# WilliamFlinchbaugh/Deep-RL-Battlespace

Measured on AMD Instinct MI355X. Metric: agent-steps/sec, higher is better.
Workload: dtype f64/i16

## Files before the change

### deep-rl-battlespace_amd/build.py

```python
import os
import subprocess
import sys

HERE = os.path.dirname(os.path.abspath(__file__))
CSRC = os.path.join(HERE, "csrc")
INCLUDE = os.path.join(os.path.dirname(HERE), "include")
LIB = os.path.join(CSRC, "libbattlespace_hip.so")
COMMON = ["-O3", "--offload-arch=gfx950", "-fPIC", "-std=c++17", "-Wall", "-Wno-unused-function"]
STEP_FLAGS = ["-ffp-contract=off", "-mllvm", "-disable-machine-licm", "-mllvm", "-amdgpu-mfma-vgpr-form", "-mllvm", "-amdgpu-kernarg-preload-count=15"]
PER_CALL_FLAGS = STEP_FLAGS + ["-mllvm", "-amdgpu-sched-strategy=max-ilp"]
SOURCES = [(os.path.join(CSRC, "bsx_kernels.hip"), STEP_FLAGS),
           (os.path.join(CSRC, "bsx_step_per_call.hip"), PER_CALL_FLAGS),
           (os.path.join(CSRC, "bsx_step_multi_tick.hip"), STEP_FLAGS),
           (os.path.join(CSRC, "bsx_step_two_wave.hip"), PER_CALL_FLAGS),
           (os.path.join(CSRC, "bsx_step_rollout.hip"), STEP_FLAGS),
           (os.path.join(CSRC, "bsx_actor.hip"), ["-ffp-contract=off", "-mllvm", "-amdgpu-mfma-vgpr-form"]),
           (os.path.join(CSRC, "bsx_actor_grad.hip"), ["-ffp-contract=off", "-mllvm", "-amdgpu-mfma-vgpr-form"]),
           (os.path.join(CSRC, "bsx_replay.hip"), []),
           (os.path.join(CSRC, "bsx_advantage.hip"), ["-ffp-contract=off"]),
           (os.path.join(CSRC, "bsx_ppo_head.hip"), []),
           (os.path.join(CSRC, "bsx_adam_step.hip"), [])]


def _stale():
    if not os.path.exists(LIB):
        return True
    t = os.path.getmtime(LIB)
    import glob
    deps = [src for src, _ in SOURCES] + glob.glob(os.path.join(CSRC, "*.h")) + glob.glob(os.path.join(CSRC, "*.inl")) + \
        [os.path.join(INCLUDE, "battlespace_hip.h"), os.path.abspath(__file__)]
    return any(os.path.getmtime(d) > t for d in deps)


def build(force=False, verbose=False):
    if not force and not _stale():
        return LIB
    hipcc = os.environ.get("HIPCC", "/opt/rocm/bin/hipcc")
    from concurrent.futures import ThreadPoolExecutor

    def compile_one(item):
        src, extra = item
        obj = os.path.splitext(src)[0] + ".o"
        cmd = [hipcc, *COMMON, *extra, "-I", INCLUDE, "-c", src, "-o", obj]
        if verbose:
            print(" ".join(cmd), flush=True)
        subprocess.run(cmd, check=True)
        return obj
    with ThreadPoolExecutor(max_workers=len(SOURCES)) as pool:
        objs = list(pool.map(compile_one, SOURCES))
    cmd = [hipcc, "--offload-arch=gfx950", "-shared", "-fPIC", *objs, "-o", LIB]
    if verbose:
        print(" ".join(cmd), flush=True)
    subprocess.run(cmd, check=True)
    return LIB


if __name__ == "__main__":
    print(build(force="--force" in sys.argv, verbose=True))
```

### deep-rl-battlespace_amd/csrc/bsx_kernels.hip

```cpp

#include <array>
#include <mutex>
#include <unordered_map>

#include "bsx_config.h"
#include "bsx_args.h"
#include "bsx_state.h"
#include "bsx_rng.h"
#include "bsx_geometry.h"
#include "bsx_instinct.h"
#include "bsx_step_kernel.h"
#define BSX_INST_PER_CALL
#define BSX_INST_MULTI_TICK
#define BSX_INST_ROLLOUT
#include "bsx_step_split.h"
#define BSX_INST_SPLIT_MANY
#define BSX_INST_SPLIT
#define BSX_INST_SPLIT_CONT
#ifdef BSX_VARIANT
#define BSX_INST_KW
#else
#define BSX_INST_KW extern
#endif
#include "bsx_step_instances.h"
using namespace bsxk;

namespace {

struct ResetArgs {
    StatePtrs st; int64_t E; int n; const uint8_t* mask; const int32_t* spawn; uint64_t seed; uint64_t nonce;
    int64_t env_offset; float* obs; int observe_only;
};

__global__ __launch_bounds__(TPB) void bsx_reset_kernel(const ResetArgs p) {
    const int n = p.n, A = 2 * n, G = group_width(n), EPB = TPB / G;
    const int tid = threadIdx.x, a = tid & (G - 1), gl = tid & ~(G - 1);
    const int64_t e = int64_t(blockIdx.x) * EPB + (tid / G);
    const bool env_ok = e < p.E, valid = env_ok && a < A;
    const size_t g = valid ? size_t(e) * A + a : 0;
    __shared__ volatile int s_x[TPB], s_y[TPB], s_hp[TPB];

    EnvU er = {};
    uint32_t games = 0;
    int x = 0, y = 0, hp = 0;
    double dir = 0.0;
    bool frac = false;
    if (env_ok) {
        const uint2 dw = p.st.envd[e];
        er = unpack_env(p.st.envc[e], dw.x);
        games = dw.y;
    }
    if (valid) {
        const uint2 pw = p.st.plane[g];
        unpack_plane(pw, x, y, hp, dir);
        frac = (pw.y & PLANE_FRAC) != 0u;
        if (frac) dir = p.st.pdirf[g];
    }
    const bool doit = env_ok && !p.observe_only && (!p.mask || p.mask[e]);
    if (p.spawn) {
        if (doit) {
            const int32_t* s = p.spawn + size_t(e) * (4 + 3 * A);
            er.brx = s[0]; er.bry = s[1]; er.bbx = s[2]; er.bby = s[3];
            if (valid) { x = s[4 + 3 * a]; y = s[5 + 3 * a]; dir = double(s[6 + 3 * a]); }
        }
    } else if (!p.observe_only) {
        const int64_t genv = p.env_offset + (env_ok ? e : p.E - 1);
        const int ac = a < A ? a : A - 1;
        const SpawnDraw sd = spawn_from_words(draw4(p.seed, genv, STREAM_RESET, uint32_t(p.nonce), uint32_t(ac)), ac, n);
        const int lane0 = (tid & 63) & ~(G - 1);
        const int rbx = __shfl(sd.bx, lane0), rby = __shfl(sd.by, lane0), bbx = __shfl(sd.bx, lane0 + n), bby = __shfl(sd.by, lane0 + n);
        if (doit) {
            er.brx = rbx; er.bry = rby; er.bbx = bbx; er.bby = bby;
            if (valid) { x = sd.x; y = sd.y; dir = double(sd.dir); }
        }
    }
    if (doit) {
        er.bhp_r = er.bhp_b = 5 * n;
        er.tick = 0; er.done = 0; er.winner = BSX_WINNER_NONE;
        hp = PLANE_HP; frac = false;
        if (valid) p.st.plane[g] = pack_plane(x, y, hp, dir, false);
        if (valid && a == 0) { p.st.envc[e] = pack_envc(er); p.st.envd[e] = make_uint2(pack_envd(er), games); }
    }
    if (!p.observe_only) {
        const int lane = tid & 63;
        const int64_t wb = int64_t(blockIdx.x) * (TPB / 64) + (tid >> 6);
        const unsigned long long resetting = __ballot(doit);
        if (resetting != 0ull && wb < wave_blocks(p.E, n)) {
            uint2* const pool = p.st.bent + size_t(wb) * POOL_CAP;
            const int pc = int(p.st.bcnt[wb]);
            int wpos = 0;
            for (int base = 0; base < pc; base += 64) {
                const int w = base + lane;
                const uint2 en = pool[w < pc ? w : 0];
                const bool stay = w < pc && ((resetting >> (en.x >> ENT_OWNER_SHIFT)) & 1ull) == 0ull;
                const unsigned long long kb = __ballot(stay);
                const int ps = wpos + __popcll(kb & ((1ull << lane) - 1ull));
                if (stay) pool[ps] = en;
                wpos += __popcll(kb);
            }
            if (lane == 0) p.st.bcnt[wb] = uint32_t(wpos);
        }
    }
    s_x[tid] = x; s_y[tid] = y; s_hp[tid] = valid ? hp : 0;
    __syncthreads();
    if (valid && p.obs) {
        const int team = a < n ? 0 : 1;
        write_obs<0>(p.obs + g * size_t(3 * n + 2), n, hp > 0, x, y, dir, a,
                     team == 0 ? er.bbx : er.brx, team == 0 ? er.bby : er.bry, gl, s_x, s_y, s_hp);
    }
}

__global__ void bsx_mark_done_kernel(uint2* envd, int64_t E) {
    const int64_t e = int64_t(blockIdx.x) * blockDim.x + threadIdx.x;
    if (e < E) envd[e] = make_uint2(1u << 27, 0u);
}

struct ExportArgs { StatePtrs st; int64_t E; int n; BsxExport out; int tie_tick; };

__global__ __launch_bounds__(TPB) void bsx_export_kernel(const ExportArgs p) {
    const int A = 2 * p.n;
    const size_t EA = size_t(p.E) * A;
    const size_t g = size_t(blockIdx.x) * TPB + threadIdx.x;
    if (g >= EA) return;
    const int64_t e = int64_t(g / A);
    const int a = int(g % A);
    const uint2 pw = p.st.plane[g];
    int x, y, hp;
    double dir;
    unpack_plane(pw, x, y, hp, dir);
    if (pw.y & PLANE_FRAC) dir = p.st.pdirf[g];
    const BsxExport& o = p.out;
    if (o.px) o.px[g] = x;
    if (o.py) o.py[g] = y;
    if (o.pdir) o.pdir[g] = dir;
    if (o.php) o.php[g] = hp;
    if (o.palive) o.palive[g] = hp > 0;
    const uint2 dw = p.st.envd[e];
    const EnvU ev = unpack_env(p.st.envc[e], dw.x);
    const int ptick = ev.tick - ((ev.done && ev.winner == BSX_WINNER_TIE && ev.tick >= p.tie_tick) ? 1 : 0);
    for (int k = 0; k < K; ++k) {
        const size_t i = g * K + k;
        if (o.bl_live) o.bl_live[i] = 0;
        if (o.bl_x) o.bl_x[i] = 0;
        if (o.bl_y) o.bl_y[i] = 0;
        if (o.bl_dir) o.bl_dir[i] = 0.0;
    }
    const int G = group_width(p.n), EPB = 64 / G;
    const int64_t wb = e / EPB;
    const uint32_t me = uint32_t(int(e % EPB) * G + a);
    const uint2* const pool = p.st.bent + size_t(wb) * POOL_CAP;
    const int cnt = int(p.st.bcnt[wb]);
    for (int j2 = 0; j2 < cnt; ++j2) {
        const uint32_t w = pool[j2].x;
        const int age = bullet_age(w);
        if ((w >> ENT_OWNER_SHIFT) != me || age == int(TOMBSTONE_AGE)) continue;
        int slot = (ptick - age + 1) % K;
        if (slot < 0) slot += K;
        const size_t i = g * K + slot;
        if (o.bl_live) o.bl_live[i] = 1;
        if (o.bl_x) o.bl_x[i] = bullet_x(w);
        if (o.bl_y) o.bl_y[i] = bullet_y(w);
        if (o.bl_dir) o.bl_dir[i] = p.st.bdir[size_t(slot) * EA + g];
    }
    if (a == 0) {
        if (o.base_xy) { o.base_xy[4 * e] = ev.brx; o.base_xy[4 * e + 1] = ev.bry; o.base_xy[4 * e + 2] = ev.bbx; o.base_xy[4 * e + 3] = ev.bby; }
        if (o.bhp) { o.bhp[2 * e] = ev.bhp_r; o.bhp[2 * e + 1] = ev.bhp_b; }
        if (o.tick) o.tick[e] = ev.tick;
        if (o.env_done) o.env_done[e] = ev.done;
        if (o.winner) o.winner[e] = ev.winner;
        if (o.counters) {
            const int* c4 = p.st.cnt + 4 * e;
            o.counters[4 * e] = c4[0]; o.counters[4 * e + 1] = c4[1]; o.counters[4 * e + 2] = c4[2]; o.counters[4 * e + 3] = c4[3];
        }
    }
}

struct InstinctArgs {
    const float* obs; void* actions; const double* rnd; int64_t E; int n; int team; int out_kind; int continuous;
    uint64_t seed; uint64_t seq; const uint64_t* seq_base; int64_t env_offset;
};

__global__ __launch_bounds__(TPB) void bsx_instinct_kernel(const InstinctArgs p) {
    const int A = 2 * p.n, D = 3 * p.n + 2;
    const size_t g = size_t(blockIdx.x) * TPB + threadIdx.x;
    if (g >= size_t(p.E) * A) return;
    const int a = int(g % A);
    const int tm = a < p.n ? 0 : 1;
    if (p.team != 2 && p.team != tm) return;
    const float* o = p.obs + g * D;
    double td, ta;
    const int act = instinct_choose([&](int k) { return o[k]; }, p.n, td, ta);
    if (!p.continuous) {
        if (p.out_kind == BSX_ACT_I32) static_cast<int32_t*>(p.actions)[g] = act;
        else static_cast<float4*>(p.actions)[g] = one_hot_scores(act);
        return;
    }
    double r0, n0, n1, n2;
    if (p.rnd) { r0 = p.rnd[4 * g]; n0 = p.rnd[4 * g + 1]; n1 = p.rnd[4 * g + 2]; n2 = p.rnd[4 * g + 3]; }
    else instinct_continuous_draws(p.seed, p.seq + (p.seq_base ? *p.seq_base : 0ull), uint64_t(p.env_offset) * uint64_t(A) + g, r0, n0, n1, n2);
    double* out = static_cast<double*>(p.actions) + 3 * g;
    instinct_continuous_action(td, ta, r0, n0, n1, n2, out[0], out[1], out[2]);
}

std::mutex g_family_mu;
std::unordered_map<const void*, int> g_family;
inline void family_forget(const void* state) {
    std::lock_guard<std::mutex> lk(g_family_mu);
    g_family.erase(state);
}
inline bool family_claim(const void* state, bool cont) {
    std::lock_guard<std::mutex> lk(g_family_mu);
    int& f = g_family[state];
    if (f == 0) f = cont ? 2 : 1;
    return f == (cont ? 2 : 1);
}
inline int grid_for(int64_t E, int n) {
    const int epb = TPB / group_width(n);
    return int((E + epb - 1) / epb);
}

inline bool narrow_offsets_ok(int64_t E, int n, uint32_t flags) {
    return !(flags & BSX_F_WIDE_OFFSETS) && uint64_t(E) * uint64_t(2 * n) * 200ull <= 0xFFFFFFFFull;
}
constexpr int64_t SPLIT_MAX_GAMES = 114688, SPLIT_MANY_MAX_GAMES = 65536, SPLIT_CONT_MAX_GAMES = 81920;
constexpr int64_t SPLIT_DRAW_MAX_GAMES = 98304;
constexpr int64_t SPLIT_MANY_FORM2_FROM = 32768;
template <bool CONT, bool MULTI>
inline bool split_applies(int n, const StepArgs& a, int64_t bound) {
    if (n != 1 || (a.flags & BSX_F_ONE_WAVE)) return false;
    if (CONT) return !MULTI && bound <= SPLIT_CONT_MAX_GAMES;
    return bound <= (MULTI ? SPLIT_MANY_MAX_GAMES : SPLIT_MAX_GAMES);
}

using StepKernel = void (*)(BSX_STEP_KERNEL_PARAMS);

template <class F>
StepKernel by_team_and_offsets(int n, bool off32, F f) {
    const auto w = [&](auto N) { return off32 ? f(N, std::true_type{}) : f(N, std::false_type{}); };
    switch (n) {
        case 1: return w(std::integral_constant<int, 1>{});
        case 2: return w(std::integral_constant<int, 2>{});
        case 3: return w(std::integral_constant<int, 3>{});
        case 4: return w(std::integral_constant<int, 4>{});
        default: return w(std::integral_constant<int, 0>{});
    }
}

template <bool CONT, bool MULTI, bool ACTOR, bool LG>
int launch_for_n(const StepArgs& a, int64_t bound, void* stream) {
    const int n = a.n;
    const bool two_wave = !ACTOR && split_applies<CONT, MULTI>(n, a, bound);
    const StepKernel k = by_team_and_offsets(n, narrow_offsets_ok(a.E, n, a.flags), [&](auto N_, auto OFF32_) -> StepKernel {
        constexpr int N = decltype(N_)::value;
        constexpr bool OFF32 = decltype(OFF32_)::value;
        if constexpr (ACTOR) {
            if constexpr (N == 0) return nullptr;
            else return bsx_step_kernel<N, CONT, true, true, false, OFF32>;
        } else {
            if constexpr (N == 1 && !(CONT && MULTI)) {
                if (two_wave) {
                    if constexpr (MULTI)
                        return bound > SPLIT_MANY_FORM2_FROM ? bsx_step_split_kernel<LG, OFF32, 2>
                                                             : bsx_step_split_kernel<LG, OFF32, 1>;
                    else if constexpr (CONT)
                        return bsx_step_split_kernel<false, OFF32, 0, true, true>;
                    else
                        return bound <= SPLIT_DRAW_MAX_GAMES ? bsx_step_split_kernel<LG, OFF32, 0, false, true>
                                                             : bsx_step_split_kernel<LG, OFF32, 0>;
                }
            }
            return bsx_step_kernel<N, CONT, MULTI, false, LG, OFF32>;
        }
    });
    const StepGeometry geo = step_geometry(ACTOR ? FORM_ROLLOUT : (two_wave ? FORM_TWO_WAVE : FORM_ONE_WAVE), bound, n);
    const dim3 grid(unsigned(geo.groups));
    const dim3 block(SPB * geo.waves);
    hipLaunchKernelGGL(k, grid, block, 0, static_cast<hipStream_t>(stream),
                       bound, a.st.envc, a.st.envd, a.st.plane, a.actions, a.st.bent, a.st.bcnt, a.action_kind, a);
    return int(hipGetLastError());
}

StepArgs step_args(void* state, int64_t E, int n, int T, float* rew, uint8_t* done, uint8_t* env_done, uint8_t* winner,
                   uint8_t* env_done_t, const BsxRewards* cfg, uint32_t flags, uint64_t seed, int64_t env_offset) {
    StepArgs a{};
    a.st = state_ptrs(state, E, n);
    a.E = E; a.n = n; a.T = T;
    a.rew = rew; a.done = done; a.env_done = env_done; a.winner = winner; a.env_done_t = env_done_t;
    a.cfg = *cfg; a.flags = flags; a.seed = seed; a.env_offset = env_offset; a.tie_tick = tie_tick_const(n);
    a.scripted_team = -1;
    return a;
}

struct StepCall { int64_t first = 0, count = -1; int T = 0; int store_all = 0; uint8_t* env_done_t = nullptr; };

template <bool CONT>
int step(const StepCall& c, void* state, int64_t E, int n, const void* actions, int action_kind, const double* u, float* obs, float* rew,
         uint8_t* done, uint8_t* env_done, uint8_t* winner, const BsxRewards* cfg, uint32_t flags, uint64_t seed, int64_t env_offset,
         void* stream) {
    const int T = c.T;
    const int64_t first = c.first, count = c.count < 0 ? E - first : c.count;
    if (T < 0 || T > BSX_MAX_T || first < 0 || count <= 0 || first > E - count || (first & 255) || ((first || count != E) && T != 0))
        return BSX_E_ARG;
    if (!obs || !rew || !done || !cfg || (!actions && (T || !(flags & BSX_F_EMPTY_CALL)))) return BSX_E_ARG;
    if (const int rc = check_games(state, E, n)) return rc;
    if (!aligned(obs, 4) || !aligned(rew, 4) || (u && !aligned(u, 8))) return BSX_E_ALIGN;
    if (!CONT && action_kind == BSX_ACT_LOGITS_F32 && !aligned(actions, 16)) return BSX_E_ALIGN;
    if (!CONT && action_kind != BSX_ACT_I32 && action_kind != BSX_ACT_LOGITS_F32) return BSX_E_ARG;
    if (CONT && action_kind != BSX_ACT_F32 && action_kind != BSX_ACT_F64 && action_kind != BSX_ACT_F32X4) return BSX_E_ARG;
    if (CONT && action_kind == BSX_ACT_F32X4 && !aligned(actions, 16)) return BSX_E_ALIGN;
    if (!family_claim(state, CONT)) return BSX_E_FAMILY;
    StepArgs a = step_args(state, E, n, T, rew, done, env_done, winner, c.env_done_t, cfg, flags, seed, env_offset);
    a.actions = actions; a.action_kind = action_kind; a.u = u; a.obs = obs;
    if (!actions) { a.actions = state; a.action_kind = -1; }
    const int64_t EA = E * 2 * n;
    a.act_tb = EA * (CONT ? (action_kind == BSX_ACT_F32 ? 12 : (action_kind == BSX_ACT_F64 ? 24 : 16)) : (action_kind == BSX_ACT_I32 ? 4 : 16));
    a.u_ts = EA;
    a.obs_ts = c.store_all ? EA * (3 * n + 2) : 0; a.rew_ts = c.store_all ? EA : 0; a.done_ts = c.store_all ? EA : 0;
    if (first) {
        const int64_t fa = first * 2 * n;
        const int64_t fb = first / (64 / group_width(n));
        a.st.envc += first; a.st.envd += first; a.st.cnt += 4 * first; a.st.plane += fa; a.st.pdirf += fa;
        a.st.bcnt += fb; a.st.bent += fb * POOL_CAP; a.st.bdir += fa; a.st.bd += fa;
        if (actions) a.actions = static_cast<const char*>(actions) + fa * (a.act_tb / EA);
        if (u) a.u += fa;
        a.obs += fa * (3 * n + 2); a.rew += fa; a.done += fa;
        if (env_done) a.env_done += first;
        if (winner) a.winner += first;
        a.env_offset += first;
    }
    const bool lg = !CONT && action_kind == BSX_ACT_LOGITS_F32;
    if (T == 0) return lg ? launch_for_n<CONT, false, false, !CONT>(a, count, stream) : launch_for_n<CONT, false, false, false>(a, count, stream);
    return lg ? launch_for_n<CONT, true, false, !CONT>(a, count, stream) : launch_for_n<CONT, true, false, false>(a, count, stream);
}

template <bool CONT>
int rollout(void* state, int64_t E, int n, int T, const float* weights, int precision, int scripted_team, uint64_t scripted_seed, float* obs,
            float* scores, float* rew, uint8_t* done, uint8_t* env_done, uint8_t* winner, uint8_t* env_done_t, const BsxRewards* cfg,
            uint32_t flags, const BsxActorNoise* noise, uint64_t actor_seed, uint64_t seq, const uint64_t* seq_base, uint64_t seed,
            int64_t env_offset, void* stream, bool gauss = false, const BsxGaussianHead* head = nullptr) {
    if (T < 1 || T > BSX_MAX_T || !weights || !obs || !scores || !rew || !done || !cfg || (flags & BSX_F_EMPTY_CALL) ||
        (precision != BSX_ACTOR_F32 && precision != BSX_ACTOR_BF16X3 && precision != BSX_ACTOR_BF16X6) || scripted_team < -1 || scripted_team > 1)
        return BSX_E_ARG;
    if (gauss && (!head || !head->log_std)) return BSX_E_ARG;
    if (const int rc = check_games(state, E, n, 256, ROLLOUT_MAX_N)) return rc;
    if (!aligned(weights, 16) || !aligned(scores, 16) || !aligned(obs, 4) || !aligned(rew, 4)) return BSX_E_ALIGN;
    BsxActorNoise nz = {};
    if (noise) nz = *noise;
    if (gauss) {
        if (nz.gaussian_std > 0.f || nz.ou_scale > 0.f || nz.sample_mode != 0 || nz.u_inject || nz.logp) return BSX_E_ARG;
        if (!aligned(head->log_std, 4) || (head->logp && !aligned(head->logp, 4))) return BSX_E_ALIGN;
    }
    if (nz.ou_scale > 0.f && (!nz.ou_state || !aligned(nz.ou_state, 16))) return nz.ou_state ? BSX_E_ALIGN : BSX_E_ARG;
    if (nz.z_inject || nz.u_inject) return BSX_E_ARG;
    if (nz.sample_mode != 0 && (nz.sample_mode != 1 || !(nz.temperature > 0.f) || CONT)) return BSX_E_ARG;
    if ((nz.logp && !aligned(nz.logp, 4)) || (nz.value_weights && !aligned(nz.value_weights, 16))) return BSX_E_ALIGN;
    if (nz.value_weights && (n != 1 || !nz.value || !aligned(nz.value, 4))) return BSX_E_ARG;
    if (!family_claim(state, CONT)) return BSX_E_FAMILY;
    const int64_t EA = E * 2 * n, D = 3 * n + 2;
    StepArgs a = step_args(state, E, n, T, rew, done, env_done, winner, env_done_t, cfg, flags, seed, env_offset);
    a.action_kind = CONT ? BSX_ACT_F32X4 : BSX_ACT_LOGITS_F32;
    a.obs = obs + EA * D; a.obs_ts = EA * D; a.rew_ts = EA; a.done_ts = EA;
    a.aw = weights; a.aprec = precision; a.scripted_team = scripted_team; a.obs0 = obs; a.scores = scores; a.scores_ts = EA * 4; a.nz = nz;
    a.aseed = actor_seed; a.aseq = seq; a.aseq_base = seq_base; a.iseed = scripted_seed;
    if (gauss) a.gh = *head;
    return launch_for_n<CONT, true, true, false>(a, E, stream);
}

const std::array<double2, 361>& heading_table() {
    static const std::array<double2, 361> lut = [] {
        std::array<double2, 361> t;
        const double st = 215 * 0.1;
        for (int d = 0; d <= 360; ++d) {
            const double ang = -(double(d) * DEG2RAD);
            t[d].x = st * cos(ang);
            t[d].y = st * sin(ang);
        }
        return t;
    }();
    return lut;
}

}

extern "C" {

int bsx_abi_version(void) { return BSX_ABI_VERSION; }

int bsx_build_flags(void) { return BUILD_FLAGS; }

int bsx_stream_synchronize(void* stream) { return int(hipStreamSynchronize(static_cast<hipStream_t>(stream))); }

int bsx_host_device_pointer(void* host, void** device) {
    if (!host || !device) return BSX_E_ARG;
    return int(hipHostGetDevicePointer(device, host, 0));
}

int bsx_tie_tick(int n) { return tie_tick_const(n); }

int bsx_state_bytes(int64_t E, int n, size_t* bytes) {
    if (const int rc = check_games(bytes, E, n, 1)) return rc;
    *bytes = make_layout(E, n).total;
    return 0;
}

int bsx_state_init(void* state, int64_t E, int n, void* stream) {
    if (const int rc = check_games(state, E, n)) return rc;
    const Layout L = make_layout(E, n);
    family_forget(state);
    hipStream_t s = static_cast<hipStream_t>(stream);
    hipError_t err = hipMemsetAsync(state, 0, L.total, s);
    if (err != hipSuccess) return int(err);
    const std::array<double2, 361>& lut = heading_table();
    err = hipMemcpyAsync(static_cast<char*>(state) + L.lut, lut.data(), sizeof(double2) * lut.size(), hipMemcpyHostToDevice, s);
    if (err != hipSuccess) return int(err);
    hipLaunchKernelGGL(bsx_mark_done_kernel, dim3(unsigned((E + TPB - 1) / TPB)), dim3(TPB), 0, s,
                       reinterpret_cast<uint2*>(static_cast<char*>(state) + L.envd), E);
    return int(hipGetLastError());
}

int bsx_state_release(void* state) {
    if (!state) return BSX_E_ARG;
    family_forget(state);
    return 0;
}

int bsx_reset(void* state, int64_t E, int n, const uint8_t* reset_mask, const int32_t* spawn, uint64_t seed,
              uint64_t nonce, int64_t env_offset, float* obs, void* stream) {
    if (const int rc = check_games(state, E, n)) return rc;
    if ((spawn && !aligned(spawn, 4)) || (obs && !aligned(obs, 4))) return BSX_E_ALIGN;
    if (!reset_mask) family_forget(state);
    ResetArgs a{state_ptrs(state, E, n), E, n, reset_mask, spawn, seed, nonce, env_offset, obs, 0};
    hipLaunchKernelGGL(bsx_reset_kernel, dim3(grid_for(E, n)), dim3(TPB), 0, static_cast<hipStream_t>(stream), a);
    return int(hipGetLastError());
}

int bsx_step_discrete(void* state, int64_t E, int n, const void* actions, int action_kind, const double* u, float* obs,
                      float* rew, uint8_t* done, uint8_t* env_done, uint8_t* winner, const BsxRewards* cfg,
                      uint32_t flags, uint64_t seed, int64_t env_offset, void* stream) {
    return step<false>({}, state, E, n, actions, action_kind, u, obs, rew, done, env_done, winner, cfg, flags, seed, env_offset, stream);
}

int bsx_step_continuous(void* state, int64_t E, int n, const void* actions, int action_kind, const double* u,
                        float* obs, float* rew, uint8_t* done, uint8_t* env_done, uint8_t* winner,
                        const BsxRewards* cfg, uint32_t flags, uint64_t seed, int64_t env_offset, void* stream) {
    return step<true>({}, state, E, n, actions, action_kind, u, obs, rew, done, env_done, winner, cfg, flags, seed, env_offset, stream);
}

int bsx_step_discrete_range(void* state, int64_t E, int n, int64_t first, int64_t count, const void* actions, int action_kind, const double* u,
                            float* obs, float* rew, uint8_t* done, uint8_t* env_done, uint8_t* winner, const BsxRewards* cfg,
                            uint32_t flags, uint64_t seed, int64_t env_offset, void* stream) {
    return step<false>({first, count}, state, E, n, actions, action_kind, u, obs, rew, done, env_done, winner, cfg, flags, seed, env_offset, stream);
}

int bsx_step_continuous_range(void* state, int64_t E, int n, int64_t first, int64_t count, const void* actions, int action_kind, const double* u,
                              float* obs, float* rew, uint8_t* done, uint8_t* env_done, uint8_t* winner, const BsxRewards* cfg,
                              uint32_t flags, uint64_t seed, int64_t env_offset, void* stream) {
    return step<true>({first, count}, state, E, n, actions, action_kind, u, obs, rew, done, env_done, winner, cfg, flags, seed, env_offset, stream);
}

int bsx_step_many_discrete(void* state, int64_t E, int n, int T, const void* actions, int action_kind, const double* u,
                           float* obs, float* rew, uint8_t* done, uint8_t* env_done, uint8_t* winner, uint8_t* env_done_t, const BsxRewards* cfg,
                           uint32_t flags, int store_all, uint64_t seed, int64_t env_offset, void* stream) {
    return T < 1 ? BSX_E_ARG : step<false>({0, -1, T, store_all, env_done_t}, state, E, n, actions, action_kind, u, obs, rew, done, env_done,
                                           winner, cfg, flags, seed, env_offset, stream);
}

int bsx_step_many_continuous(void* state, int64_t E, int n, int T, const void* actions, int action_kind, const double* u,
                             float* obs, float* rew, uint8_t* done, uint8_t* env_done, uint8_t* winner, uint8_t* env_done_t, const BsxRewards* cfg,
                             uint32_t flags, int store_all, uint64_t seed, int64_t env_offset, void* stream) {
    return T < 1 ? BSX_E_ARG : step<true>({0, -1, T, store_all, env_done_t}, state, E, n, actions, action_kind, u, obs, rew, done, env_done,
                                          winner, cfg, flags, seed, env_offset, stream);
}

int bsx_rollout_discrete(void* state, int64_t E, int n, int T, const float* weights, int precision, int scripted_team, float* obs, float* scores, float* rew,
                         uint8_t* done, uint8_t* env_done, uint8_t* winner, uint8_t* env_done_t, const BsxRewards* cfg, uint32_t flags,
                         const BsxActorNoise* noise, uint64_t actor_seed, uint64_t seq, const uint64_t* seq_base, uint64_t seed,
                         int64_t env_offset, void* stream) {
    return rollout<false>(state, E, n, T, weights, precision, scripted_team, 0, obs, scores, rew, done, env_done, winner, env_done_t, cfg, flags,
                          noise, actor_seed, seq, seq_base, seed, env_offset, stream);
}

int bsx_rollout_continuous(void* state, int64_t E, int n, int T, const float* weights, int precision, int scripted_team, uint64_t scripted_seed, float* obs, float* scores, float* rew,
                           uint8_t* done, uint8_t* env_done, uint8_t* winner, uint8_t* env_done_t, const BsxRewards* cfg, uint32_t flags,
                           const BsxActorNoise* noise, uint64_t actor_seed, uint64_t seq, const uint64_t* seq_base, uint64_t seed,
                           int64_t env_offset, void* stream) {
    return rollout<true>(state, E, n, T, weights, precision, scripted_team, scripted_seed, obs, scores, rew, done, env_done, winner, env_done_t, cfg, flags,
                         noise, actor_seed, seq, seq_base, seed, env_offset, stream);
}

int bsx_rollout_continuous_gaussian(void* state, int64_t E, int n, int T, const float* weights, int precision, int scripted_team,
                                    uint64_t scripted_seed, float* obs, float* scores, float* rew,
                                    uint8_t* done, uint8_t* env_done, uint8_t* winner, uint8_t* env_done_t, const BsxRewards* cfg,
                                    uint32_t flags, const BsxActorNoise* noise, const BsxGaussianHead* head, uint64_t actor_seed,
                                    uint64_t seq, const uint64_t* seq_base, uint64_t seed, int64_t env_offset, void* stream) {
    return rollout<true>(state, E, n, T, weights, precision, scripted_team, scripted_seed, obs, scores, rew, done, env_done, winner, env_done_t, cfg, flags,
                         noise, actor_seed, seq, seq_base, seed, env_offset, stream, true, head);
}

__global__ void bsx_selftest_atan2_kernel(int R, unsigned long long* out) {
    const int W = 2 * R + 1;
    const long long total = (long long)W * W;
    unsigned long long bad = 0, seen = 0;
    for (long long i = (long long)blockIdx.x * blockDim.x + threadIdx.x; i < total; i += (long long)gridDim.x * blockDim.x) {
        const int iy = int(i / W) - R, ix = int(i % W) - R;
        const double lib = atan2(double(iy), double(ix));
        const double one = atan2_pixels(iy, ix);
        const int ys[3] = {iy, ix, -iy}, xs[3] = {ix, iy, ix};
        double three[3];
        atan2_pixels_n<3>(ys, xs, three);
        const bool ok = __double_as_longlong(one) == __double_as_longlong(lib) && __double_as_longlong(three[0]) == __double_as_longlong(lib) &&
                        __double_as_longlong(three[1]) == __double_as_longlong(atan2(double(ix), double(iy))) &&
                        __double_as_longlong(three[2]) == __double_as_longlong(atan2(double(-iy), double(ix)));
        bad += ok ? 0ull : 1ull;
        seen += 1ull;
    }
    atomicAdd(&out[0], bad); atomicAdd(&out[1], seen);
}
int bsx_selftest_atan2(int R, uint64_t* out, void* stream) {
    if (!out || R < 0 || R > 4096) return BSX_E_ARG;
    hipStream_t st = static_cast<hipStream_t>(stream);
    hipError_t err = hipMemsetAsync(out, 0, 2 * sizeof(uint64_t), st);
    if (err != hipSuccess) return int(err);
    bsx_selftest_atan2_kernel<<<1024, 256, 0, st>>>(R, reinterpret_cast<unsigned long long*>(out));
    return int(hipGetLastError());
}

int bsx_observe(void* state, int64_t E, int n, float* obs, void* stream) {
    if (!obs) return BSX_E_ARG;
    if (const int rc = check_games(state, E, n)) return rc;
    if (!aligned(obs, 4)) return BSX_E_ALIGN;
    ResetArgs a{state_ptrs(state, E, n), E, n, nullptr, nullptr, 0, 0, 0, obs, 1};
    hipLaunchKernelGGL(bsx_reset_kernel, dim3(grid_for(E, n)), dim3(TPB), 0, static_cast<hipStream_t>(stream), a);
    return int(hipGetLastError());
}

int bsx_export_state(const void* state, int64_t E, int n, const BsxExport* out, void* stream) {
    if (!out) return BSX_E_ARG;
    if (const int rc = check_games(state, E, n)) return rc;
    ExportArgs a{state_ptrs(const_cast<void*>(state), E, n), E, n, *out, bsx_tie_tick(n)};
    const size_t EA = size_t(E) * 2 * n;
    hipLaunchKernelGGL(bsx_export_kernel, dim3(unsigned((EA + TPB - 1) / TPB)), dim3(TPB), 0,
                       static_cast<hipStream_t>(stream), a);
    return int(hipGetLastError());
}

int bsx_instinct_discrete(const float* obs, void* actions, int out_kind, int64_t E, int n, int team, void* stream) {
    if (!actions || team < 0 || team > 2 || (out_kind != BSX_ACT_I32 && out_kind != BSX_ACT_LOGITS_F32)) return BSX_E_ARG;
    if (const int rc = check_games(obs, E, n, 4)) return rc;
    if (!aligned(actions, out_kind == BSX_ACT_I32 ? 4 : 16)) return BSX_E_ALIGN;
    InstinctArgs a{obs, actions, nullptr, E, n, team, out_kind, 0, 0, 0, nullptr, 0};
    const size_t EA = size_t(E) * 2 * n;
    hipLaunchKernelGGL(bsx_instinct_kernel, dim3(unsigned((EA + TPB - 1) / TPB)), dim3(TPB), 0, static_cast<hipStream_t>(stream), a);
    return int(hipGetLastError());
}

int bsx_instinct_continuous_shard(const float* obs, double* actions, const double* rnd, int64_t E, int n, int team,
                                  uint64_t seed, uint64_t seq, const uint64_t* seq_base, int64_t env_offset, void* stream) {
    if (!actions || team < 0 || team > 2 || env_offset < 0) return BSX_E_ARG;
    if (const int rc = check_games(obs, E, n, 4)) return rc;
    if (!aligned(actions, 8) || (rnd && !aligned(rnd, 8))) return BSX_E_ALIGN;
    InstinctArgs a{obs, actions, rnd, E, n, team, 0, 1, seed, seq, seq_base, env_offset};
    const size_t EA = size_t(E) * 2 * n;
    hipLaunchKernelGGL(bsx_instinct_kernel, dim3(unsigned((EA + TPB - 1) / TPB)), dim3(TPB), 0, static_cast<hipStream_t>(stream), a);
    return int(hipGetLastError());
}

int bsx_instinct_continuous(const float* obs, double* actions, const double* rnd, int64_t E, int n, int team,
                            uint64_t seed, uint64_t seq, const uint64_t* seq_base, void* stream) {
    return bsx_instinct_continuous_shard(obs, actions, rnd, E, n, team, seed, seq, seq_base, 0, stream);
}

}
```

### deep-rl-battlespace_amd/csrc/bsx_step_kernel.h

```cpp
#pragma once

namespace bsxk {

__device__ inline int argmax4(float a, float b, float c, float d) {
    int am = 0;
    float best = a;
    const float v[3] = {b, c, d};
#pragma unroll
    for (int i = 0; i < 3; ++i)
        if (!(best != best) && (v[i] > best || v[i] != v[i])) { am = i + 1; best = v[i]; }
    return am;
}

struct StepArgs {
    StatePtrs st;
    int64_t E; int n;
    const void* actions; int action_kind;
    const double* u;
    float* obs; float* rew; uint8_t* done; uint8_t* env_done; uint8_t* winner;
    uint8_t* env_done_t;
    BsxRewards cfg;
    uint32_t flags; uint64_t seed; int64_t env_offset; int tie_tick;
    int T; int64_t act_tb , u_ts, obs_ts, rew_ts, done_ts ;
    const float* aw; int aprec; int scripted_team ; const float* obs0; float* scores; int64_t scores_ts; BsxActorNoise nz; uint64_t aseed, aseq; const uint64_t* aseq_base;
    uint64_t iseed;
    BsxGaussianHead gh;
};

#define BSX_STEP_KERNEL_PARAMS                                                                                                           \
    const int64_t E_, const uint2* const envc_, const uint2* const envd_, const uint2* const plane_, const void* const act_,               \
        const uint2* const bent_, const uint32_t* const bcnt_, const int kind_, const bsxk::StepArgs p_

template <int N>
__device__ inline void write_obs(float* __restrict__ out, int n, bool alive, int x, int y, double dir, int a,
                                 int ebx, int eby, int gl, const volatile int* s_x, const volatile int* s_y,
                                 const volatile int* s_hp) {
    const int D = 3 * n + 2;
    if (!alive || (DIAG & 1u)) {
        for (int i = 0; i < D; ++i) out[i] = -1.0f;
        return;
    }
    out[0] = obs_dist(x, y, ebx, eby);
    out[1] = obs_angle(x, y, dir, ebx, eby);
    const int eb = gl + (a < n ? n : 0);
    for (int j = 0; j < n; ++j) {
        if (s_hp[eb + j] > 0) {
            const int qx = s_x[eb + j], qy = s_y[eb + j];
            out[2 + 3 * j] = 1.0f;
            out[3 + 3 * j] = obs_dist(x, y, qx, qy);
            out[4 + 3 * j] = obs_angle(x, y, dir, qx, qy);
        } else {
            out[2 + 3 * j] = -1.0f; out[3 + 3 * j] = -1.0f; out[4 + 3 * j] = -1.0f;
        }
    }
}

enum Mode : int { M_INERT = 0, M_TIE = 1, M_PHYS = 2, M_RESET = 3 };

constexpr int tie_tick_const(int n) {
    const double max_time = double(10 + n * 2);
    double t = 0.0;
    int k = 0;
    do { t += 0.1; ++k; } while (!(t >= max_time));
    return k;
}
static_assert(tie_tick_const(1) == 121 && tie_tick_const(2) == 141 && tie_tick_const(3) == 161 && tie_tick_const(4) == 181 &&
              tie_tick_const(5) == 200, "time-limit tick");
static_assert(tie_tick_const(BSX_MAX_N) < 512, "the game clock fits the 9 bits of the game record");

template <class T> __device__ inline T* elem(T* base, uint32_t i) {
    typedef typename std::conditional<std::is_const<T>::value, const char, char>::type byte_t;
    return reinterpret_cast<T*>(reinterpret_cast<byte_t*>(base) + uint32_t(i * uint32_t(sizeof(T))));
}
template <class T> __device__ inline T* elem(T* base, size_t i) { return base + i; }
__device__ inline void end_of_tick() {
    __builtin_amdgcn_fence(__ATOMIC_RELEASE, "wavefront");
    __builtin_amdgcn_wave_barrier();
    __builtin_amdgcn_fence(__ATOMIC_ACQUIRE, "wavefront");
}
template <int N, bool CONT, bool MULTI, bool ACTOR = false, bool LG = false, bool OFF32 = false>
__global__ __launch_bounds__(SPB * (ACTOR ? group_width(N > 0 ? N : 1) / 2 : WPB)) __attribute__((amdgpu_waves_per_eu((ACTOR && N > 1) ? 2 : ((!ACTOR && MULTI && N == 2) ? 4 : 1))))
void bsx_step_kernel(BSX_STEP_KERNEL_PARAMS) {
    const StepArgs& p = p_;
    const unsigned stamp_row = blockIdx.x; (void)stamp_row;
    STAMP(8);
    typedef typename std::conditional<OFF32, uint32_t, size_t>::type ix_t;
    typedef typename std::conditional<OFF32, int32_t, int64_t>::type ixs_t;
    constexpr bool NT_STATE = !MULTI && N >= 2;
    constexpr int WAVES = ACTOR ? group_width(N > 0 ? N : 1) / 2 : WPB;
    const int n = (N > 0) ? N : p.n;
    const int A = 2 * n;
    const int G = group_width(n);
    const int EPB = SPB / G;
    const int wave = (WAVES > 1) ? int(threadIdx.x >> 6) : 0;
    const int tid = (WAVES > 1) ? int(threadIdx.x & 63) : int(threadIdx.x);
    const ixs_t wblk = (WAVES > 1) ? ixs_t(blockIdx.x) * WAVES + wave : ixs_t(blockIdx.x);
    const int a = tid & (G - 1);
    const ixs_t e = wblk * EPB + (tid / G);
    const bool env_ok = e < ixs_t(E_);
    const bool valid = env_ok && a < A;
    const ix_t EA = ix_t((MULTI || ACTOR) ? E_ : p.E) * ix_t(A);
    const ixs_t ec = env_ok ? e : ixs_t(E_ - 1);
    const ix_t g = ix_t(ec) * A + (a < A ? a : A - 1);
    constexpr int MANY = -1; constexpr bool DRAW = false;
#include "bsx_step_lds.inl"

    const bool has_act = kind_ >= 0;
    struct RawIn { int ai; float4 lg; float f0, f1, f2; double c0, c1, c2, uu; };
    auto load_inputs = [&](int t, RawIn& r) {
        const void* const at = MULTI ? static_cast<const void*>(static_cast<const char*>(act_) + int64_t(t) * p.act_tb) : act_;
        const double* const ut = (MULTI && p.u) ? p.u + int64_t(t) * p.u_ts : p.u;
        if (!CONT) {
            const char* const abase = static_cast<const char*>(at);
            if constexpr (LG) r.lg = *reinterpret_cast<const float4*>(elem(abase, has_act ? g * 16 : ix_t(0)));
            else r.ai = *reinterpret_cast<const int32_t*>(elem(abase, has_act ? g * 4 : ix_t(0)));
        } else if (has_act) {
            if (kind_ == BSX_ACT_F32) {
                const float* ap = static_cast<const float*>(at) + 3 * g;
                r.f0 = ap[0]; r.f1 = ap[1]; r.f2 = ap[2];
            } else if (kind_ == BSX_ACT_F32X4) {
                const float4 v = static_cast<const float4*>(at)[g];
                r.f0 = v.x; r.f1 = v.y; r.f2 = v.z;
            } else {
                const double* ap = static_cast<const double*>(at) + 3 * g;
                r.c0 = ap[0]; r.c1 = ap[1]; r.c2 = ap[2];
            }
        }
        __builtin_amdgcn_sched_barrier(0);
        if (ut) r.uu = ut[g];
    };
    int x = 0, y = 0, hp = 0;
    uint32_t games = 0;
    double dir = 0.0;
    EnvU er = {};
    const ix_t pool0 = ix_t(wblk) * ix_t(POOL_CAP);
    uint32_t pc = 0;
    uint2 pool_first = make_uint2(0u, 0u);
    RawIn rin = {}, rin_next = {};
    struct DecIn { int act; double a0, a1, a2, uu; };
    auto decode = [&](const RawIn& r) {
        DecIn d = {-1, 0.0, 0.0, 0.0, 0.0};
        if (has_act) {
            if (!CONT) {
                if constexpr (!LG) d.act = r.ai;
                else d.act = argmax4(r.lg.x, r.lg.y, r.lg.z, r.lg.w);
            } else if (kind_ == BSX_ACT_F32 || kind_ == BSX_ACT_F32X4) {
                d.a0 = double(r.f0); d.a1 = double(r.f1); d.a2 = double(r.f2);
            } else {
                d.a0 = r.c0; d.a1 = r.c1; d.a2 = r.c2;
            }
        }
        if (p.u) d.uu = r.uu;
        return d;
    };
    DecIn din_next = {-1, 0.0, 0.0, 0.0, 0.0};
    if (MULTI && !ACTOR) { load_inputs(0, rin_next); din_next = decode(rin_next); }
    if constexpr (ACTOR) {
        constexpr int D = 3 * N + 2;
        for (int i = int(threadIdx.x); i < 2 * N * bsx_actor::SMALL / 4; i += SPB * WAVES) {
            const int ag = i / (bsx_actor::SMALL / 4), j = i - ag * (bsx_actor::SMALL / 4);
            reinterpret_cast<float4*>(s_small)[i] =
                reinterpret_cast<const float4*>(p.aw + size_t(ag) * bsx_actor::blob_floats(D) + bsx_actor::off_small(D))[j];
        }
        if constexpr (N == 1) {
            if (p.nz.value_weights)
                for (int i = int(threadIdx.x); i < 2 * bsx_actor::SMALL / 4; i += SPB * WAVES) {
                    const int ag = i / (bsx_actor::SMALL / 4), j = i - ag * (bsx_actor::SMALL / 4);
                    reinterpret_cast<float4*>(s_small + 2 * bsx_actor::SMALL)[i] =
                        reinterpret_cast<const float4*>(p.nz.value_weights + size_t(ag) * bsx_actor::blob_floats(D) + bsx_actor::off_small(D))[j];
                }
        }
        const int64_t e_first = wblk * EPB;
        const int64_t nfl = min(int64_t(SPB), (E_ - e_first) * A) * D;
        if (G == A) {
            for (int i = tid; i < SPB * D; i += SPB) s_obs[i] = i < nfl ? p.obs0[size_t(e_first) * A * D + i] : -1.0f;
        } else {
            for (int k = 0; k < D; ++k) s_obs[tid * D + k] = valid ? p.obs0[g * D + k] : -1.0f;
        }
        __builtin_amdgcn_fence(__ATOMIC_RELEASE, "workgroup");
        if (WAVES > 1) __syncthreads(); else __builtin_amdgcn_wave_barrier();
        __builtin_amdgcn_fence(__ATOMIC_ACQUIRE, "workgroup");
    }

    for (int tk = 0; tk < (MULTI ? p.T : 1); ++tk) {
    ix_t gt = g, EAt = EA;
    uint64_t seed_t = p.seed;
    int64_t env_offset_t = p.env_offset;
    constexpr int TIE_C = tie_tick_const(N > 0 ? N : 1);
    int tie_tick = (N > 0) ? TIE_C : p.tie_tick;
    if (MULTI) {
        asm volatile("" : "+v"(gt));
        asm volatile("" : "+s"(EAt));
        asm volatile("" : "+s"(seed_t));
    }
    int tid_k = tid;
    if constexpr ((ACTOR && N > 1) || (MULTI && !ACTOR && N > 0 && ((OPAQUE_MULTI_MASK >> (((LG || CONT) ? 8 : 0) + N)) & 1))) asm volatile("" : "+v"(tid_k));
    typedef const StepArgs __attribute__((address_space(4))) StepArgsK;
    static_assert(alignof(StepArgs) == 8, "kernarg offset of StepArgs");
    const char __attribute__((address_space(4)))* ka = (const char __attribute__((address_space(4)))*)__builtin_amdgcn_kernarg_segment_ptr();
    if (MULTI) asm volatile("" : "+s"(ka));
    auto& p = [&]() -> decltype(auto) { if constexpr (MULTI) return (*reinterpret_cast<StepArgsK*>(ka + 64)); else return (p_); }();
    const int tid = tid_k, lane = tid, a = tid & (G - 1);
    const int gl = tid & ~(G - 1);
    const int team = (a < n) ? 0 : 1;
    const int eb = gl + (team == 0 ? n : 0);
    const double* const u_t = (MULTI && p.u) ? p.u + int64_t(tk) * p.u_ts : p.u;
    float* const obs_t = MULTI ? p.obs + int64_t(tk) * p.obs_ts : p.obs;
    float* const rew_t = MULTI ? p.rew + int64_t(tk) * p.rew_ts : p.rew;
    uint8_t* const done_t = MULTI ? p.done + int64_t(tk) * p.done_ts : p.done;
    STAMP(0);
    if (!MULTI || tk == 0) {
        const uint2 ecw = *elem(envc_, ix_t(ec));
        const uint2 edw = *elem(envd_, ix_t(ec));
        const uint2 prw = *elem(plane_, gt);
        double dirf = 0.0;
        pool_first = *elem(bent_, pool0 + ix_t(lane));
        if (!(DIAG & 2u)) pc = __builtin_amdgcn_readfirstlane(*elem(bcnt_, ix_t(wblk)));
        if constexpr (CONT) dirf = *elem(p.st.pdirf, gt);
        if (!MULTI) load_inputs(0, rin);
        if (!MULTI) {
            asm volatile("" : "+s"(seed_t), "+s"(env_offset_t));
            if (N == 0) asm volatile("" : "+s"(tie_tick));
        }
        unpack_plane(prw, x, y, hp, dir);
        if constexpr (CONT) dir = (prw.y & PLANE_FRAC) ? dirf : dir;
        er = unpack_env(ecw, edw.x);
        games = edw.y;
    } else {
        pool_first = *elem(bent_, pool0 + ix_t(lane));
    }
    const DecIn din = MULTI ? din_next : decode(rin);
    int act = din.act;
    double a0 = din.a0, a1 = din.a1, a2 = din.a2, uu_in = din.uu;
    constexpr bool R_BULLETS = true, R_MOVE = true, R_STAGE = true, R_GEOM = true, R_OUTCOME = true, R_ST_STATE = true, R_ST_OUT = true, R_POSE_LDS = false;
    constexpr int R_RDV_COUNTS = 0, R_GEOM_LDS = 0, R_PUB = 0, R_DRAW_LDS = 0;
    auto split_rendezvous = [] {};
#include "bsx_step_phase_actor.inl"
#include "bsx_step_phase_shot.inl"
#include "bsx_step_phase_move.inl"
#include "bsx_step_phase_geometry.inl"
#include "bsx_step_phase_bullets.inl"
#include "bsx_step_phase_outcome.inl"
#include "bsx_step_phase_stores.inl"
    STAMP(7);
    if (MULTI) {
        games += uint32_t(cnt_delta.x);
        end_of_tick();
        STAMP(9);
    }
    }
}

}
```

### deep-rl-battlespace_amd/csrc/bsx_step_split.h

```cpp
#pragma once

namespace bsxk {

template <bool LG, bool OFF32, int MANY = 0, bool CONT_ = false, bool DRAW = false>
__global__ __launch_bounds__(2 * SPB)
void bsx_step_split_kernel(BSX_STEP_KERNEL_PARAMS) {
    constexpr int N = 1;
    constexpr bool CONT = CONT_, MULTI = MANY != 0, ACTOR = false;
    static_assert(!CONT || (MANY == 0 && !LG), "continuous actions: the per-call form only");
    static_assert(!DRAW || MANY == 0, "the geometry wave's draw: the per-call form only");
    const StepArgs& p = p_;
    typedef typename std::conditional<OFF32, uint32_t, size_t>::type ix_t;
    typedef typename std::conditional<OFF32, int32_t, int64_t>::type ixs_t;
    constexpr bool NT_STATE = false;
    constexpr int WAVES = 1;
    const int n = 1, A = 2, G = 2, EPB = SPB / 2;
    const int wave = 0;
    const int role_wave = int(threadIdx.x >> 6);
    const unsigned stamp_row = blockIdx.x * 2u + unsigned(role_wave); (void)stamp_row;
    STAMP(8);
    STAMP_HWID();
    const int tid = int(threadIdx.x & 63);
    const ixs_t wblk = ixs_t(blockIdx.x);
    const int a = tid & (G - 1);
    const ixs_t e = wblk * EPB + (tid / G);
    const bool env_ok = e < ixs_t(E_);
    const bool valid = env_ok && a < A;
    const ix_t EA = ix_t(MULTI ? E_ : p.E) * ix_t(A);
    const ixs_t ec = env_ok ? e : ixs_t(E_ - 1);
    const ix_t g = ix_t(ec) * A + (a < A ? a : A - 1);
#include "bsx_step_lds.inl"
    auto split_rendezvous = [] {
        asm volatile("s_waitcnt lgkmcnt(0)\n\ts_barrier" ::: "memory");
    };
    const bool has_act = kind_ >= 0;
    struct RawIn { int ai; float4 lg; double uu; };
    struct DecIn { int act; double uu; };
    auto load_inputs = [&](int t, RawIn& r) {
        const char* const abase = static_cast<const char*>(act_) + (MULTI ? int64_t(t) * p.act_tb : int64_t(0));
        if constexpr (LG) r.lg = *reinterpret_cast<const float4*>(elem(abase, has_act ? g * 16 : ix_t(0)));
        else r.ai = *reinterpret_cast<const int32_t*>(elem(abase, has_act ? g * 4 : ix_t(0)));
        __builtin_amdgcn_sched_barrier(0);
        const double* const ut = (MULTI && p.u) ? p.u + int64_t(t) * p.u_ts : p.u;
        if (ut) r.uu = ut[g];
    };
    auto decode = [&](const RawIn& r) {
        DecIn d = {-1, 0.0};
        if (has_act) d.act = LG ? argmax4(r.lg.x, r.lg.y, r.lg.z, r.lg.w) : r.ai;
        if (p.u) d.uu = r.uu;
        return d;
    };
    const ix_t pool0 = ix_t(wblk) * ix_t(POOL_CAP);
    if constexpr (MANY != 0) {
        if (role_wave == 0) {
            __builtin_amdgcn_s_setprio(1);
            constexpr bool R_BULLETS = true, R_MOVE = true, R_STAGE = true, R_GEOM = false, R_OUTCOME = true, R_POSE_LDS = false;
            constexpr bool R_ST_STATE = MANY == 2, R_ST_OUT = false;
            constexpr int R_RDV_COUNTS = MANY == 2 ? 0 : 1, R_GEOM_LDS = 0, R_PUB = MANY == 2 ? 1 : 0, R_DRAW_LDS = 0;
            s_ov[tid] = 0ull;
#include "bsx_step_split_many_body.inl"
        } else if constexpr (MANY == 2) {
            constexpr bool R_BULLETS = false, R_GEOM = true, R_ST_STATE = false, R_ST_OUT = true;
            constexpr int R_GEOM_LDS = 0, R_PUB = 0;
#include "bsx_step_split_out_body.inl"
        } else {
            constexpr bool R_BULLETS = false, R_MOVE = true, R_STAGE = false, R_GEOM = true, R_OUTCOME = true, R_POSE_LDS = false;
            constexpr bool R_ST_STATE = true, R_ST_OUT = true;
            constexpr int R_RDV_COUNTS = 2, R_GEOM_LDS = 0, R_PUB = 0, R_DRAW_LDS = 0;
#include "bsx_step_split_many_body.inl"
        }
    } else {
        constexpr int R_PUB = 0;
        const int tk = 0;
        if (role_wave == 0) {
            __builtin_amdgcn_s_setprio(1);
            constexpr bool R_BULLETS = true, R_MOVE = true, R_STAGE = true, R_GEOM = false, R_OUTCOME = true, R_ST_STATE = true, R_ST_OUT = true;
            constexpr bool R_POSE_LDS = true;
            constexpr int R_RDV_COUNTS = 0, R_GEOM_LDS = 2, R_DRAW_LDS = DRAW ? 2 : 0;
            s_ov[tid] = 0ull;
#include "bsx_step_split_body.inl"
        } else {
#include "bsx_step_split_geom_body.inl"
        }
    }
}

}
```

Baseline: 23.93 billion.

## Pack kernel arguments into preloaded dwords and reorder continuous action loads

Shrinks the bound to int32 and packs action kind and team size into one dword, so the leading kernel arguments exactly fill 14 preloaded SGPR dwords and the StepArgs block follows at a fixed offset. The per-call path reads n from the preloaded argument instead of the argument block. Continuous actions are now fetched with a unified 12-byte vector load issued before the direction load, and the jitter load is split from the action load. Per-tick pointer computations are moved later. This adds a host-side bound check and relies on the environment count fitting in 32 bits.

```diff
diff --git a/deep-rl-battlespace_amd/build.py b/deep-rl-battlespace_amd/build.py
--- a/deep-rl-battlespace_amd/build.py
+++ b/deep-rl-battlespace_amd/build.py
@@ -7,7 +7,7 @@
 INCLUDE = os.path.join(os.path.dirname(HERE), "include")
 LIB = os.path.join(CSRC, "libbattlespace_hip.so")
 COMMON = ["-O3", "--offload-arch=gfx950", "-fPIC", "-std=c++17", "-Wall", "-Wno-unused-function"]
-STEP_FLAGS = ["-ffp-contract=off", "-mllvm", "-disable-machine-licm", "-mllvm", "-amdgpu-mfma-vgpr-form", "-mllvm", "-amdgpu-kernarg-preload-count=15"]
+STEP_FLAGS = ["-ffp-contract=off", "-mllvm", "-disable-machine-licm", "-mllvm", "-amdgpu-mfma-vgpr-form", "-mllvm", "-amdgpu-kernarg-preload-count=14"]
 PER_CALL_FLAGS = STEP_FLAGS + ["-mllvm", "-amdgpu-sched-strategy=max-ilp"]
 SOURCES = [(os.path.join(CSRC, "bsx_kernels.hip"), STEP_FLAGS),
            (os.path.join(CSRC, "bsx_step_per_call.hip"), PER_CALL_FLAGS),
diff --git a/deep-rl-battlespace_amd/csrc/bsx_kernels.hip b/deep-rl-battlespace_amd/csrc/bsx_kernels.hip
--- a/deep-rl-battlespace_amd/csrc/bsx_kernels.hip
+++ b/deep-rl-battlespace_amd/csrc/bsx_kernels.hip
@@ -248,6 +248,7 @@
 
 template <bool CONT, bool MULTI, bool ACTOR, bool LG>
 int launch_for_n(const StepArgs& a, int64_t bound, void* stream) {
+    if (bound > (int64_t(1) << 30)) return BSX_E_ARG;
     const int n = a.n;
     const bool two_wave = !ACTOR && split_applies<CONT, MULTI>(n, a, bound);
     const StepKernel k = by_team_and_offsets(n, narrow_offsets_ok(a.E, n, a.flags), [&](auto N_, auto OFF32_) -> StepKernel {
@@ -276,7 +277,7 @@
     const dim3 grid(unsigned(geo.groups));
     const dim3 block(SPB * geo.waves);
     hipLaunchKernelGGL(k, grid, block, 0, static_cast<hipStream_t>(stream),
-                       bound, a.st.envc, a.st.envd, a.st.plane, a.actions, a.st.bent, a.st.bcnt, a.action_kind, a);
+                       int32_t(bound), pack_kind_n(a.action_kind, n), a.st.envc, a.st.envd, a.st.plane, a.actions, a.st.bent, a.st.bcnt, a);
     return int(hipGetLastError());
 }
 
diff --git a/deep-rl-battlespace_amd/csrc/bsx_step_kernel.h b/deep-rl-battlespace_amd/csrc/bsx_step_kernel.h
--- a/deep-rl-battlespace_amd/csrc/bsx_step_kernel.h
+++ b/deep-rl-battlespace_amd/csrc/bsx_step_kernel.h
@@ -28,8 +28,16 @@
 };
 
 #define BSX_STEP_KERNEL_PARAMS                                                                                                           \
-    const int64_t E_, const uint2* const envc_, const uint2* const envd_, const uint2* const plane_, const void* const act_,               \
-        const uint2* const bent_, const uint32_t* const bcnt_, const int kind_, const bsxk::StepArgs p_
+    const int32_t E_, const int32_t kind_n_, const uint2* const envc_, const uint2* const envd_, const uint2* const plane_,               \
+        const void* const act_, const uint2* const bent_, const uint32_t* const bcnt_, const bsxk::StepArgs p_
+inline int32_t pack_kind_n(int action_kind, int n) { return int32_t((uint32_t(action_kind) & 0xFFFFu) | (uint32_t(n) << 16)); }
+__device__ inline int packed_kind(int32_t kind_n) { return int(int16_t(kind_n)); }
+__device__ inline int packed_n(int32_t kind_n) { return int(kind_n >> 16); }
+static_assert(BSX_MAX_N < (1 << 15), "the team size fits the upper half of the packed argument");
+constexpr int STEP_KERNEL_PRELOAD_DWORDS = 14;
+constexpr int STEP_ARGS_KERNARG_OFFSET = 2 * 4 + 6 * 8;
+static_assert(STEP_ARGS_KERNARG_OFFSET == 4 * STEP_KERNEL_PRELOAD_DWORDS && STEP_ARGS_KERNARG_OFFSET % alignof(StepArgs) == 0,
+              "the leading arguments fill the preloadable dwords exactly and the argument block follows without padding");
 
 template <int N>
 __device__ inline void write_obs(float* __restrict__ out, int n, bool alive, int x, int y, double dir, int a,
@@ -73,6 +81,18 @@
     return reinterpret_cast<T*>(reinterpret_cast<byte_t*>(base) + uint32_t(i * uint32_t(sizeof(T))));
 }
 template <class T> __device__ inline T* elem(T* base, size_t i) { return base + i; }
+typedef uint32_t u32x3_t __attribute__((ext_vector_type(3)));
+typedef u32x3_t u32x3_a4_t __attribute__((aligned(4)));
+template <class IX>
+__device__ inline void load_cont_action(const void* act, IX g, int kind, bool has_act, float& f0, float& f1, float& f2, double& c0,
+                                        double& c1, double& c2) {
+    const uint32_t stride = kind == BSX_ACT_F32 ? 12u : (kind == BSX_ACT_F32X4 ? 16u : 24u);
+    const char* const ap = elem(static_cast<const char*>(act), has_act ? g * IX(stride) : IX(0));
+    const u32x3_t w0 = *reinterpret_cast<const u32x3_a4_t*>(ap);
+    const u32x3_t w1 = *reinterpret_cast<const u32x3_a4_t*>(ap + (kind == BSX_ACT_F64 ? 12 : 0));
+    f0 = __uint_as_float(w0.x); f1 = __uint_as_float(w0.y); f2 = __uint_as_float(w0.z);
+    c0 = __hiloint2double(int(w0.y), int(w0.x)); c1 = __hiloint2double(int(w1.x), int(w0.z)); c2 = __hiloint2double(int(w1.z), int(w1.y));
+}
 __device__ inline void end_of_tick() {
     __builtin_amdgcn_fence(__ATOMIC_RELEASE, "wavefront");
     __builtin_amdgcn_wave_barrier();
@@ -82,15 +102,16 @@
 __global__ __launch_bounds__(SPB * (ACTOR ? group_width(N > 0 ? N : 1) / 2 : WPB)) __attribute__((amdgpu_waves_per_eu((ACTOR && N > 1) ? 2 : ((!ACTOR && MULTI && N == 2) ? 4 : 1))))
 void bsx_step_kernel(BSX_STEP_KERNEL_PARAMS) {
     const StepArgs& p = p_;
+    const int kind_ = packed_kind(kind_n_);
     const unsigned stamp_row = blockIdx.x; (void)stamp_row;
     STAMP(8);
     typedef typename std::conditional<OFF32, uint32_t, size_t>::type ix_t;
     typedef typename std::conditional<OFF32, int32_t, int64_t>::type ixs_t;
     constexpr bool NT_STATE = !MULTI && N >= 2;
     constexpr int WAVES = ACTOR ? group_width(N > 0 ? N : 1) / 2 : WPB;
-    const int n = (N > 0) ? N : p.n;
+    const int n = (N > 0) ? N : (MULTI ? p.n : packed_n(kind_n_));
     const int A = 2 * n;
-    const int G = group_width(n);
+    const int G = (N > 0 || MULTI) ? group_width(n) : (1 << (32 - __builtin_clz(unsigned(2 * n - 1))));
     const int EPB = SPB / G;
     const int wave = (WAVES > 1) ? int(threadIdx.x >> 6) : 0;
     const int tid = (WAVES > 1) ? int(threadIdx.x & 63) : int(threadIdx.x);
@@ -99,7 +120,7 @@
     const ixs_t e = wblk * EPB + (tid / G);
     const bool env_ok = e < ixs_t(E_);
     const bool valid = env_ok && a < A;
-    const ix_t EA = ix_t((MULTI || ACTOR) ? E_ : p.E) * ix_t(A);
+    const ix_t EA = ix_t((MULTI || ACTOR) ? int64_t(E_) : p.E) * ix_t(A);
     const ixs_t ec = env_ok ? e : ixs_t(E_ - 1);
     const ix_t g = ix_t(ec) * A + (a < A ? a : A - 1);
     constexpr int MANY = -1; constexpr bool DRAW = false;
@@ -107,13 +128,14 @@
 
     const bool has_act = kind_ >= 0;
     struct RawIn { int ai; float4 lg; float f0, f1, f2; double c0, c1, c2, uu; };
-    auto load_inputs = [&](int t, RawIn& r) {
+    auto load_action = [&](int t, RawIn& r) {
         const void* const at = MULTI ? static_cast<const void*>(static_cast<const char*>(act_) + int64_t(t) * p.act_tb) : act_;
-        const double* const ut = (MULTI && p.u) ? p.u + int64_t(t) * p.u_ts : p.u;
         if (!CONT) {
             const char* const abase = static_cast<const char*>(at);
             if constexpr (LG) r.lg = *reinterpret_cast<const float4*>(elem(abase, has_act ? g * 16 : ix_t(0)));
             else r.ai = *reinterpret_cast<const int32_t*>(elem(abase, has_act ? g * 4 : ix_t(0)));
+        } else if constexpr (!MULTI) {
+            load_cont_action(at, g, kind_, has_act, r.f0, r.f1, r.f2, r.c0, r.c1, r.c2);
         } else if (has_act) {
             if (kind_ == BSX_ACT_F32) {
                 const float* ap = static_cast<const float*>(at) + 3 * g;
@@ -126,8 +148,15 @@
                 r.c0 = ap[0]; r.c1 = ap[1]; r.c2 = ap[2];
             }
         }
+    };
+    auto load_jitter = [&](int t, RawIn& r) {
+        const double* const ut = (MULTI && p.u) ? p.u + int64_t(t) * p.u_ts : p.u;
+        if (ut) r.uu = ut[g];
+    };
+    auto load_inputs = [&](int t, RawIn& r) {
+        load_action(t, r);
         __builtin_amdgcn_sched_barrier(0);
-        if (ut) r.uu = ut[g];
+        load_jitter(t, r);
     };
     int x = 0, y = 0, hp = 0;
     uint32_t games = 0;
@@ -171,7 +200,7 @@
                 }
         }
         const int64_t e_first = wblk * EPB;
-        const int64_t nfl = min(int64_t(SPB), (E_ - e_first) * A) * D;
+        const int64_t nfl = min(int64_t(SPB), (int64_t(E_) - e_first) * A) * D;
         if (G == A) {
             for (int i = tid; i < SPB * D; i += SPB) s_obs[i] = i < nfl ? p.obs0[size_t(e_first) * A * D + i] : -1.0f;
         } else {
@@ -199,15 +228,11 @@
     static_assert(alignof(StepArgs) == 8, "kernarg offset of StepArgs");
     const char __attribute__((address_space(4)))* ka = (const char __attribute__((address_space(4)))*)__builtin_amdgcn_kernarg_segment_ptr();
     if (MULTI) asm volatile("" : "+s"(ka));
-    auto& p = [&]() -> decltype(auto) { if constexpr (MULTI) return (*reinterpret_cast<StepArgsK*>(ka + 64)); else return (p_); }();
+    auto& p = [&]() -> decltype(auto) { if constexpr (MULTI) return (*reinterpret_cast<StepArgsK*>(ka + STEP_ARGS_KERNARG_OFFSET)); else return (p_); }();
     const int tid = tid_k, lane = tid, a = tid & (G - 1);
     const int gl = tid & ~(G - 1);
     const int team = (a < n) ? 0 : 1;
     const int eb = gl + (team == 0 ? n : 0);
-    const double* const u_t = (MULTI && p.u) ? p.u + int64_t(tk) * p.u_ts : p.u;
-    float* const obs_t = MULTI ? p.obs + int64_t(tk) * p.obs_ts : p.obs;
-    float* const rew_t = MULTI ? p.rew + int64_t(tk) * p.rew_ts : p.rew;
-    uint8_t* const done_t = MULTI ? p.done + int64_t(tk) * p.done_ts : p.done;
     STAMP(0);
     if (!MULTI || tk == 0) {
         const uint2 ecw = *elem(envc_, ix_t(ec));
@@ -216,8 +241,10 @@
         double dirf = 0.0;
         pool_first = *elem(bent_, pool0 + ix_t(lane));
         if (!(DIAG & 2u)) pc = __builtin_amdgcn_readfirstlane(*elem(bcnt_, ix_t(wblk)));
+        if (!MULTI) load_action(0, rin);
+        if (!MULTI) __builtin_amdgcn_sched_barrier(0);
         if constexpr (CONT) dirf = *elem(p.st.pdirf, gt);
-        if (!MULTI) load_inputs(0, rin);
+        if (!MULTI) load_jitter(0, rin);
         if (!MULTI) {
             asm volatile("" : "+s"(seed_t), "+s"(env_offset_t));
             if (N == 0) asm volatile("" : "+s"(tie_tick));
@@ -229,6 +256,10 @@
     } else {
         pool_first = *elem(bent_, pool0 + ix_t(lane));
     }
+    const double* const u_t = (MULTI && p.u) ? p.u + int64_t(tk) * p.u_ts : p.u;
+    float* const obs_t = MULTI ? p.obs + int64_t(tk) * p.obs_ts : p.obs;
+    float* const rew_t = MULTI ? p.rew + int64_t(tk) * p.rew_ts : p.rew;
+    uint8_t* const done_t = MULTI ? p.done + int64_t(tk) * p.done_ts : p.done;
     const DecIn din = MULTI ? din_next : decode(rin);
     int act = din.act;
     double a0 = din.a0, a1 = din.a1, a2 = din.a2, uu_in = din.uu;
diff --git a/deep-rl-battlespace_amd/csrc/bsx_step_split.h b/deep-rl-battlespace_amd/csrc/bsx_step_split.h
--- a/deep-rl-battlespace_amd/csrc/bsx_step_split.h
+++ b/deep-rl-battlespace_amd/csrc/bsx_step_split.h
@@ -10,6 +10,7 @@
     static_assert(!CONT || (MANY == 0 && !LG), "continuous actions: the per-call form only");
     static_assert(!DRAW || MANY == 0, "the geometry wave's draw: the per-call form only");
     const StepArgs& p = p_;
+    const int kind_ = packed_kind(kind_n_);
     typedef typename std::conditional<OFF32, uint32_t, size_t>::type ix_t;
     typedef typename std::conditional<OFF32, int32_t, int64_t>::type ixs_t;
     constexpr bool NT_STATE = false;
@@ -26,7 +27,7 @@
     const ixs_t e = wblk * EPB + (tid / G);
     const bool env_ok = e < ixs_t(E_);
     const bool valid = env_ok && a < A;
-    const ix_t EA = ix_t(MULTI ? E_ : p.E) * ix_t(A);
+    const ix_t EA = ix_t(MULTI ? int64_t(E_) : p.E) * ix_t(A);
     const ixs_t ec = env_ok ? e : ixs_t(E_ - 1);
     const ix_t g = ix_t(ec) * A + (a < A ? a : A - 1);
 #include "bsx_step_lds.inl"
```

Measured after the change: 24.27 billion (median of 6 runs). +1.4%, better.
